# microsoft/DFOL-VQA

Hardware: AMD Instinct MI355X
Metric: questions/sec (GQA programs, N=100 objects) (higher is better)
Workload: dtype f32

## Files before the change

dfol_vqa_amd/csrc/dfol_dense_wide.hip:

```cpp
#include "dfol_common.h"
#include "dfol_split.h"

#include <stdlib.h>

#include <algorithm>
#include <type_traits>

namespace {

constexpr int WD_BM = 128, WD_BK = 32, WD_XD = 3;
constexpr int WD_TILE = 2 * 128 * 4;
constexpr int WD_NMAX = 512;
constexpr size_t WD_LDS = (size_t)6 * WD_TILE * 16 + 2 * WD_NMAX * 4 + 8 * 4096;

template <int ACT, int XV, bool ROWS = false>
__global__ __launch_bounds__(512) __attribute__((amdgpu_waves_per_eu(2, 2))) void wide_h2_kernel(
    const float* __restrict__ X, int64_t ldx, const u32x4* __restrict__ Wp, const float* __restrict__ bias, float* __restrict__ Y, int64_t ldy, int M,
    int N, int K, int ksteps, int nbn, uint32_t* __restrict__ status, const int32_t* __restrict__ src_row) {
    extern __shared__ __attribute__((aligned(16))) u32x4 wd_sm[];
    constexpr int A0 = 0, B0 = 2 * WD_TILE;
    const int tid = threadIdx.x, lane = tid & 63, wave = __builtin_amdgcn_readfirstlane(tid >> 6), kh = lane >> 4, r16 = lane & 15;
    const int wm = wave >> 2, wn = wave & 3;
    const int arow = tid >> 2, aq = tid & 3;
    const int nblocks = (M + WD_BM - 1) / WD_BM, stride = gridDim.x;
    const int first = blockIdx.x;
    if (first >= nblocks) return;
    const int nmine = (nblocks - first + stride - 1) / stride;
    const int T = nmine * ksteps;

    floatx4 acc[4][8];
#pragma unroll
    for (int i = 0; i < 4; ++i)
#pragma unroll
        for (int j = 0; j < 8; ++j) acc[i][j] = floatx4{0.f, 0.f, 0.f, 0.f};

    float4 xa[WD_XD][2];
    int lb = first, lks = 0;
    const int r0 = min(lb * WD_BM + arow, M - 1);
    const float* xrow = X + (int64_t)(ROWS ? src_row[r0] : r0) * ldx + aq * 8;
    auto load_x = [&](auto set_tag) __attribute__((always_inline)) {
        constexpr int S = decltype(set_tag)::value;
        const int k = lks * WD_BK + aq * 8;
        const int c0 = min(k, K - 4) - aq * 8, c1 = min(k + 4, K - 4) - aq * 8;
        auto ld4 = [&](const float* p) __attribute__((always_inline)) {
            if (XV == 4) return *reinterpret_cast<const float4*>(p);
            const float2 lo = *reinterpret_cast<const float2*>(p), hi = *reinterpret_cast<const float2*>(p + 2);
            return make_float4(lo.x, lo.y, hi.x, hi.y);
        };
        xa[S][0] = ld4(xrow + c0);
        xa[S][1] = ld4(xrow + c1);
        if (++lks == ksteps) {
            lks = 0;
            lb += stride;
            const int64_t r = min((int64_t)lb * WD_BM + arow, (int64_t)M - 1);
            xrow = X + (ROWS ? (int64_t)src_row[r] : r) * ldx + aq * 8;
        }
    };
    u32x4 wb[4];
    int wks = 0, wh = 0;
    auto load_w = [&]() __attribute__((always_inline)) {
#pragma unroll
        for (int i = 0; i < 4; ++i) {
            const int idx = i * 512 + tid, nb = 2 * wh + idx / WD_TILE, within = idx % WD_TILE;
            wb[i] = Wp[((int64_t)min(nb, nbn - 1) * ksteps + wks) * WD_TILE + within];
        }
        if (++wh == 2) {
            wh = 0;
            if (++wks == ksteps) wks = 0;
        }
    };
    auto store_b = [&](int buf) __attribute__((always_inline)) {
#pragma unroll
        for (int i = 0; i < 4; ++i) wd_sm[B0 + buf * 2 * WD_TILE + i * 512 + tid] = wb[i];
    };
    float xmax = 0.f;
    int sks = 0;
    auto store_a = [&](auto set_tag, int buf) __attribute__((always_inline)) {
        constexpr int S = decltype(set_tag)::value;
        const int k = sks * WD_BK + aq * 8;
        const int at = A0 + buf * WD_TILE + arow * 4 + (aq ^ dfol_swz(arow));
        const float4 z = make_float4(0.f, 0.f, 0.f, 0.f);
        const float4 v0 = k < K ? xa[S][0] : z, v1 = k + 4 < K ? xa[S][1] : z;
        xmax = fmaxf(fmaxf(xmax, fabsf(v0.x)), fabsf(v0.y));
        xmax = fmaxf(fmaxf(xmax, fabsf(v0.z)), fabsf(v0.w));
        xmax = fmaxf(fmaxf(xmax, fabsf(v1.x)), fabsf(v1.y));
        xmax = fmaxf(fmaxf(xmax, fabsf(v1.z)), fabsf(v1.w));
        u32x4 ph, pl;
        dfol_split2hx8(v0, v1, ph, pl);
        wd_sm[at] = ph;
        wd_sm[at + WD_BM * 4] = pl;
        if (++sks == ksteps) sks = 0;
    };

    const int aoff = (wm * 64 + r16) * 4 + (kh ^ dfol_swz(r16));
    const int boff = (wn >> 1) * WD_TILE + ((wn & 1) * 64 + r16) * 4 + (kh ^ dfol_swz(r16));
    constexpr int PA3[3] = {1, 0, 0}, PB3[3] = {0, 1, 0};
    u32x4 afr[4][2];
    auto load_a = [&](int abuf) __attribute__((always_inline)) {
#pragma unroll
        for (int i = 0; i < 4; ++i)
#pragma unroll
            for (int p = 0; p < 2; ++p) afr[i][p] = wd_sm[A0 + abuf * WD_TILE + aoff + p * WD_BM * 4 + i * 64];
    };
    auto multiply = [&](int bbuf, auto half_tag) __attribute__((always_inline)) {
        constexpr int JB = 4 * decltype(half_tag)::value;
        const int bo = B0 + bbuf * 2 * WD_TILE + boff;
// ... 17 lines not shown
        xs[tid] = tid < nbn * 128 ? tail[tid] : 0.f;
        xs[WD_NMAX + tid] = (bias && tid < N) ? bias[tid] : 0.f;
    }
    float* stage = xs + 2 * WD_NMAX + wave * 1024;
    auto epilogue = [&](int b) __attribute__((always_inline)) {
        const int m0 = b * WD_BM + wm * 64;
#pragma unroll
        for (int h = 0; h < 2; ++h) {
            const int col = h * 256 + wn * 64 + lane;
            const float cs = xs[col], bv = xs[WD_NMAX + col];
            float* yp = Y + col;
#pragma unroll
            for (int i = 0; i < 4; ++i) {
#pragma unroll
                for (int j = 0; j < 4; ++j)
#pragma unroll
                    for (int e = 0; e < 4; ++e) {
                        stage[(4 * kh + e) * 64 + j * 16 + r16] = acc[i][4 * h + j][e];
                        acc[i][4 * h + j][e] = 0.f;
                    }
#pragma unroll 4
                for (int r = 0; r < 16; ++r) {
                    const int row = m0 + i * 16 + r;
                    const float v = dfol_act<ACT>(stage[r * 64 + lane] * cs + bv);
                    if (row < M && col < N) yp[(int64_t)row * ldy] = v;
                }
            }
        }
    };

    const std::integral_constant<int, 0> S0;
    const std::integral_constant<int, 1> S1;
    const std::integral_constant<int, 2> S2;
    load_x(S0);
    load_w();
    load_x(S1);
    load_x(S2);
    store_b(0);
    load_w();
    store_a(S0, 0);
    load_x(S0);
    __syncthreads();
    int g = 0, cks = 0, cb = first;
    auto body = [&](auto next_tag) __attribute__((always_inline)) {
        const int cur = g & 1, nxt = cur ^ 1;
        store_b(1);
        load_w();
        load_a(cur);
        multiply(0, S0);
        __syncthreads();
        store_b(0);
        load_w();
        store_a(next_tag, nxt);
        load_x(next_tag);
        multiply(1, S1);
        __syncthreads();
        ++g;
        if (++cks == ksteps) {
            epilogue(cb);
            cks = 0;
            cb += stride;
        }
    };
    while (g < T) {
        body(S1);
        if (g < T) body(S2);
        if (g < T) body(S0);
    }
    if (status != nullptr && !(xmax <= 65504.0f)) atomicOr(status, (uint32_t)DFOL_RANGE_X_OVERFLOW);
}

int wd_cus() {
    static int cus = 0;
    if (!cus) {
        hipDeviceProp_t prop;
        int dev = 0;
        if (hipGetDevice(&dev) == hipSuccess && hipGetDeviceProperties(&prop, dev) == hipSuccess) cus = prop.multiProcessorCount;
        if (cus <= 0) cus = 256;
    }
    return cus;
}

}

extern "C" int dfol_linear_wide_supported(int64_t M, int32_t N, int32_t K) {
    static const int on = getenv("DFOL_DENSE_WIDE") ? atoi(getenv("DFOL_DENSE_WIDE")) : 1;
    if (!on || N <= 256 || N > WD_NMAX || K < 4 * WD_BK || K % 4 != 0 || M >= (1ll << 31) - 256) return 0;
    if (on != 2 && N <= 384) return 0;
    const int64_t blocks = (M + WD_BM - 1) / WD_BM, rounds = (blocks + wd_cus() - 1) / wd_cus();
    return on == 2 || 4 * blocks >= 3 * rounds * wd_cus();
}

static int wd_launch(const char* name, const float* X, int64_t ldx, const int32_t* src_row, const void* W_split, const float* bias, float* Y, int64_t ldy,
                     int32_t M, int32_t N, int32_t K, int32_t act, void* stream);

extern "C" int dfol_linear_wide_h2_f32(const float* X, int64_t ldx, const void* W_split, const float* bias, float* Y, int64_t ldy, int32_t M, int32_t N,
                                       int32_t K, int32_t act, void* stream) {
    return wd_launch("linear_wide_h2", X, ldx, nullptr, W_split, bias, Y, ldy, M, N, K, act, stream);
}

// ... 42 lines not shown
```

dfol_vqa_amd/_lib.py:

```python

import ctypes
import os
import threading

import torch

_HERE = os.path.dirname(os.path.abspath(__file__))
LIB_PATH = os.environ.get("DFOL_LIB") or os.path.join(_HERE, "libdfolvqa.so")
_lib = None

TILE_SUBJECT_ROWS, TILE_OBJECT_ROWS = 0, 1
WANT_SUBJECT, WANT_OBJECT = 1, 2
RELATE_LONE_FORALL_IDENTITY, RELATE_DIAG_ABSENT = 1, 2
TILE_F32, TILE_BF16 = 0, 1
ACT_NONE, ACT_SIGMOID, ACT_ELU, ACT_LOGSIGMOID = 0, 1, 2, 3
LOGIC_AND, LOGIC_OR, LOGIC_NOT = 0, 1, 2


class DfolError(RuntimeError):
    pass


class LRUCache(object):

# ... 71 lines not shown
    "dfol_segment_or_ref_f32": [_p, _p, _i32, _p, _p],
    "dfol_pair_train_fwd_h2_f32": [_p, _i64, _i32, _p, _i64, _p, _p, _p, _i32, _p, _i64, _p, _p, _p, _i32, _i32, _p, _i32, _p, _p, _i64, _p, _p, _i64, _p],
    "dfol_select_rows_f32": [_p, _p, _p, _i32, _i32, _p, _p],
    "dfol_calib_features_f32": [_p, _i32, _p, _i32, _p, _i32, _p, _p],
    "dfol_attention_modulations_f32": [_p, _p, _p, _i64, _p, _i32, _i32, _i32, _p, _p],
    "dfol_implication_f32": [_p, _p, _p, _p, _i32, _i32, _p, _p],
    "dfol_compare_f32": [_p, _p, _p, _i32, _p, _p],
    "dfol_linear_act_f32": [_p, _i64, _p, _i64, _p, _p, _i64, _i32, _i32, _i32, _i32, _p],
    "dfol_box_positions_f32": [_p, _i64, _i32, _i32, _p, _i64, _i32, _p],
    "dfol_pair_features_f32": [_p, _i64, _i32, _p, _p, _i32, _i32, _p, _i64, _p],
    "dfol_reduce_by_question_f32": [_p, _p, _p, _i32, _i32, _i32, _p, _p],
    "dfol_filter_bwd_f32": [_p, _p, _p, _p, _p, _i32, _p, _i32, _i32, _i32, _p, _p, _p],
    "dfol_relate_bwd_f32": [_p, _p, _p, _p, _p, _p, _p, _p, _i32, _p, _p, _p, _i32, _i32, _i32, _i32, _p, _p, _p, _p],
    "dfol_linear_wgrad_slabs": [_i64, _i32, _i32],
    "dfol_linear_wgrad_f32": [_p, _i64, _p, _i64, _i64, _i32, _i32, _p, _p, _p],
    "dfol_linear_wgrad_workspace": [_i64, _i32, _i32],
    "dfol_linear_wgrad_bias_f32": [_p, _i64, _p, _i64, _i64, _i32, _i32, _p, _p, _p, _p],
    "dfol_attr_ll_bwd_f32": [_p, _p, _i64, _i32, _p, _i64, _p, _p, _p, _p, _i32, _i32, _i32, _p, _p, _i64, _p, _i64, _p, _p],
    "dfol_quantify_bwd_f32": [_p, _p, _p, _p, _p, _i32, _i32, _p, _p],
    "dfol_attr_gather_bwd_f32": [_p, _p, _p, _p, _i32, _i32, _i32, _p, _i64, _p],
    "dfol_rel_gather_bwd_f32": [_p, _p, _p, _p, _p, _i32, _i32, _i32, _i32, _p, _i64, _p],
    "dfol_option_normalize_bwd_f32": [_p, _p, _p, _i32, _p, _p, _i32, _i32, _p, _p],
    "dfol_modulate_f32": [_p, _p, _p, _p, _i32, _i32, _p, _p],
    "dfol_lstm_cell_f32": [_p, _i64, _i32, _p, _i64, _p, _p, _i64, _p, _i64, _p, _p, _i32, _i32, _p, _p, _p],
    "dfol_lstm_cell_tokens_f32": [_p, _i32, _p, _i32, _p, _p, _i64, _p, _p, _i64, _p, _i64, _p, _p, _i32, _i32, _p, _p, _p],
    "dfol_lstm_pointwise_f32": [_p, _p, _p, _i32, _i32, _p, _p, _p],
    "dfol_lstm_cell_train_f32": [_p, _i64, _i32, _p, _i64, _p, _p, _i64, _p, _i64, _p, _p, _i32, _i32, _p, _p, _p, _p],
    "dfol_lstm_cell_bwd_f32": [_p, _p, _p, _p, _p, _i32, _i32, _p, _p, _p],
    "dfol_lstm_cell_supported": [_i32, _i32],
    "dfol_calib_walk_supported": [_i32, _i32],
    "dfol_modulate_bwd_f32": [_p, _p, _p, _p, _p, _i32, _i32, _p, _p, _p],
    "dfol_attr_ll_f32": [_p, _i64, _i32, _p, _i64, _p, _p, _p, _p, _i32, _i32, _f, _p, _p],
    "dfol_attr_head_h2_f32": [_p, _i64, _i32, _p, _p, _i32, _p, _i64, _p, _p, _i32, _i32, _p, _p, _i32, _i32, _f, _p, _p],
    "dfol_pair_ll_f32": [_p, _i64, _i32, _p, _i64, _p, _p, _i64, _i32, _p, _i32, _p, _i64, _p, _p, _p, _i32, _i32, _p, _p, _p, _i32,
                         _i32, _f, _p, _p],
    "dfol_pair_pack_w2_f32": [_p, _i64, _i32, _i32, _p, _p],
    "dfol_pair_ll_packed_f32": [_p, _i64, _i32, _p, _i64, _p, _p, _p, _i32, _p, _i64, _p, _p, _p, _i32, _i32, _p, _p, _p, _i32, _i32, _f,
                                _i32, _p, _p],
    "dfol_pair_hidden1_fwd_f32": [_p, _i64, _p, _i64, _p, _i64, _p, _p, _p, _p, _i32, _i32, _i32, _p, _p, _p],
    "dfol_pair_hidden1_bwd_f32": [_p, _p, _p, _p, _p, _p, _i32, _i32, _i32, _p, _i64, _p, _i64, _p, _p],
    "dfol_pair_hidden1_bwd_recompute_supported": [_i32, _i32],
    "dfol_pair_hidden1_bwd_recompute_f32": [_p, _p, _i64, _p, _i64, _p, _p, _p, _p, _p, _i32, _i32, _i32, _p, _i64, _p, _i64, _p, _p],
    "dfol_pair_logit_fwd_f32": [_p, _i64, _i32, _p, _i64, _p, _p, _i32, _i64, _i64, _p, _p],
    "dfol_pair_logit_bwd_f32": [_p, _p, _i64, _i32, _p, _i64, _p, _i32, _p, _i64, _p, _i64, _p, _p],
    "dfol_pair_logit_bwd_sums_f32": [_p, _p, _i64, _i32, _p, _i64, _p, _i32, _p, _i64, _p, _p, _i64, _p],
    "dfol_linear_tall_supported": [_i64, _i32, _i32],
    "dfol_linear_tall_h2_f32": [_p, _i64, _p, _p, _p, _i64, _i32, _i32, _i32, _p, _p, _i64, _p, _i64, _p],
    "dfol_pair_dz_tall_f32": [_p, _i64, _p, _p, _p, _i64, _p, _p, _p, _i64, _i32, _i32, _i32, _i32, _p, _p],
    "dfol_pair_dz_tall_multi_f32": [_p, _i64, _p, _i64, _i32, _p, _p, _i64, _i32, _p, _p, _p, _i64, _i32, _i32, _i32, _i32, _p, _p],
    "dfol_linear_tall_bf16_bf16": [_p, _i64, _p, _p, _p, _i64, _i32, _i32, _i32, _p, _p, _i64, _p, _i64, _p],
    "dfol_pair_dz_tall_bf16": [_p, _i64, _p, _p, _p, _i64, _p, _p, _i64, _i32, _i32, _i32, _i32, _p],
    "dfol_linear_logit_h2_f32": [_p, _i64, _p, _p, _p, _i64, _i32, _i32, _i32, _p, _p, _i64, _p, _i64, _p],
    "dfol_pair_dz_fused_f32": [_p, _i64, _p, _p, _p, _i64, _p, _p, _p, _i64, _i32, _i32, _i32, _i32, _p],
    "dfol_pair_wgrad_fused_workspace": [_i64, _i32, _i32],
    "dfol_pair_wgrad_fused_sums_workspace": [_i64, _i32, _i32, _i32],
    "dfol_pair_wgrad_fused_sums_f32": [_p, _i64, _p, _p, _p, _i32, _p, _i64, _p, _p, _i64, _i64, _i32, _i32, _p, _p, _p, _i64, _p, _p, _p],
    "dfol_pair_wgrad_fused_sums_bf16": [_p, _i64, _p, _p, _p, _i32, _p, _i64, _p, _i64, _i64, _i32, _i32, _p, _p, _p, _i64, _p, _p, _p],
    "dfol_pair_wgrad_fused_f32": [_p, _i64, _p, _p, _p, _p, _i64, _p, _p, _i64, _i64, _i32, _i32, _p, _p, _p],
    "dfol_pair_wgrad_multi_scale_f32": [_p, _i64, _i32, _p, _p, _i32, _i64, _p, _p],
    "dfol_pair_wgrad_fused_multi_f32": [_p, _i64, _p, _i64, _i32, _p, _p, _p, _i64, _i32, _p, _p, _i64, _i64, _i32, _i32, _p, _p, _p],
    "dfol_linear_pack_w_bf16x3": [_p, _i64, _i32, _i32, _p, _p],
    "dfol_linear_act_split_f32": [_p, _i64, _p, _p, _p, _i64, _i32, _i32, _i32, _i32, _p],
    "dfol_linear_pack_w_bf16": [_p, _i64, _i32, _i32, _p, _p],
    "dfol_linear_act_bf16_f32": [_p, _i64, _p, _p, _p, _i64, _i32, _i32, _i32, _i32, _p],
    "dfol_linear_wgrad_bias_bf16": [_p, _i64, _p, _i64, _i64, _i32, _i32, _p, _p, _p, _p],
    "dfol_linear_wgrad_rows_supported": [_i32, _i32, _i64, _i64],
# ... 1334 lines not shown
```

dfol_vqa_amd/csrc/dfol_pair_h2.hip:

```cpp
#include "dfol_common.h"
#include "dfol_split.h"

#include <stdlib.h>

#include <type_traits>

#ifdef DFOL_PAIR_TRACE
__device__ long long dfol_h2_trace_buf[8 * 8 * 64];
#define TRACE(slot)                                                                                                  \
    do {                                                                                                             \
        if (trace_on && lane == 0) dfol_h2_trace_buf[(trace_blk * 8 + wave) * 64 + (slot)] = clock64();              \
    } while (0)
#else
#define TRACE(slot)
#endif

#ifndef DFOL_H2_PREFETCH
#define DFOL_H2_PREFETCH 1
#endif
#ifndef DFOL_H2_BDEPTH
#define DFOL_H2_BDEPTH 2
#endif
#ifndef DFOL_H1_BDEPTH
#define DFOL_H1_BDEPTH 4
#endif
#ifndef DFOL_H2_DMA_ASM
#define DFOL_H2_DMA_ASM 1
#endif
#ifndef DFOL_H2T_SKIP
#define DFOL_H2T_SKIP 0
#endif
#ifndef DFOL_H2_DMA_LATE
#define DFOL_H2_DMA_LATE 0
#endif


namespace {

constexpr float H2_NL2E = -1.44269504088896340736f;
constexpr int H2_CH = 32;
constexpr int H2_ROWS = 320, H2_TILES = 20;
constexpr int H2_PIECES = 2 * H2_ROWS * 4;
constexpr int H1_PIECES = H2_ROWS * 4;
constexpr float H2_AMAX = 60000.0f;
constexpr float H2_L2E = 1.44269504088896340736f;
constexpr float H2_LN2 = 0.69314718055994530942f;

__device__ __forceinline__ float h2_elu_neg(float zs) {
    const float p = __builtin_amdgcn_fmed3f(__builtin_amdgcn_exp2f(zs), 0.0f, 1.0f);
    return fmaf(p, H2_L2E, -H2_L2E);
}

__host__ __device__ __forceinline__ constexpr int h2_kperm(int kq, int e) { return 16 * (e >> 2) + 4 * kq + (e & 3); }

template <bool HI>
__device__ __forceinline__ float h2_resid(float x, uint32_t hpair) {
    float r;
    if (HI) asm("v_fma_mix_f32 %0, -%1, 1.0, %2 op_sel:[1,0,0] op_sel_hi:[1,0,0]" : "=v"(r) : "v"(hpair), "v"(x));
    else asm("v_fma_mix_f32 %0, -%1, 1.0, %2 op_sel:[0,0,0] op_sel_hi:[1,0,0]" : "=v"(r) : "v"(hpair), "v"(x));
    return r;
}

__global__ void h2_row_scale_kernel(const float* __restrict__ W2, int64_t ld_w2, int HID2, int HID1, float* __restrict__ tail) {
    const int lane = threadIdx.x & 63, r = blockIdx.x * (blockDim.x >> 6) + (threadIdx.x >> 6);
    if (r >= H2_ROWS) return;
    float m = 0.f;
// ... 432 lines not shown
        const float cx = p[0] + p[2] / 2.0f, cy = p[1] + p[3] / 2.0f;
        lox = fminf(lox, cx), hix = fmaxf(hix, cx), loy = fminf(loy, cy), hiy = fmaxf(hiy, cy);
    }
#pragma unroll
    for (int s = 32; s >= 1; s >>= 1) {
        lox = fminf(lox, __shfl_xor(lox, s, 64)), hix = fmaxf(hix, __shfl_xor(hix, s, 64));
        loy = fminf(loy, __shfl_xor(loy, s, 64)), hiy = fmaxf(hiy, __shfl_xor(hiy, s, 64));
    }
    if (lane == 0) box[0][wave] = lox, box[1][wave] = hix, box[2][wave] = loy, box[3][wave] = hiy;
    __syncthreads();
    if (t < HID1) {
#pragma unroll
        for (int w = 0; w < 8; ++w) lox = fminf(lox, box[0][w]), hix = fmaxf(hix, box[1][w]), loy = fminf(loy, box[2][w]), hiy = fmaxf(hiy, box[3][w]);
        const float* pf = reinterpret_cast<const float*>(part);
        float mu = -INFINITY, mv = -INFINITY;
        bool bad = false;
        for (int r = 0; r < R; ++r) {
            const float u = pf[(r * G + t / 4) * 4 + (t & 3)], v = pf[(r * G + (HID1 + t) / 4) * 4 + (t & 3)];
            const float ux = pf[(r * G + t / 4) * 4], vx = pf[(r * G + (HID1 + t) / 4) * 4];
            bad |= (ux != ux) | (vx != vx);
            mu = fmaxf(mu, u), mv = fmaxf(mv, v);
        }
        const float dmax = sqrtf((hix - lox) * (hix - lox) + (hiy - loy) * (hiy - loy));
        const float4 g = *reinterpret_cast<const float4*>(Wg + t * 4);
        const float geo = H2_L2E * (fabsf(g.x) * dmax + fabsf(g.y) * 1.57079632679489661923f + fabsf(g.z) + fabsf(g.w));
        const float bound = mu + mv + geo;
        if (bad || !(bound <= H2_AMAX)) atomicOr(status, (uint32_t)DFOL_RANGE_PAIR_SATURATED);
    }
}


constexpr int AH_WAVES = 4, AH_MT = 2, AH_T = AH_WAVES * 64, AH_SLOTS = AH_WAVES * AH_MT * 16, AH_CAP = 512;

template <int NB16>
__global__ __launch_bounds__(AH_T) void attr_head_h2_kernel(const float* pre1, int64_t ld_pre1, int HID1, const u32x4* __restrict__ W2h,
                                                            const float* __restrict__ b2, int HID2, const float* __restrict__ E, int64_t ld_e,
                                                            const float* __restrict__ be, const int32_t* __restrict__ obj_off, int Q, int O,
                                                            const int32_t* __restrict__ pred_q, const int32_t* __restrict__ pred_col, int P, int NS,
                                                            float dflt, float* __restrict__ ll, uint32_t* __restrict__ status) {
    constexpr int MT = AH_MT, ROWS = NB16 * 16, T = AH_T;
    static_assert(NB16 > 16 && NB16 <= H2_TILES, "geometry");
    __shared__ __attribute__((aligned(16))) u32x4 Bs[2 * H2_PIECES];
    constexpr int STAGE_FLOATS = 8192;
    __shared__ __attribute__((aligned(16))) float stage[STAGE_FLOATS];
    __shared__ int32_t ent[4][AH_CAP];
    __shared__ int ent_n;
    __shared__ int img_cnt[2];
    constexpr int SR = STAGE_FLOATS / ROWS - 2;

    const int tid = threadIdx.x, wave = __builtin_amdgcn_readfirstlane(tid >> 6), lane = tid & 63, kh = lane >> 4, r16 = lane & 15;
    const int nchunk = HID1 / H2_CH;
    const float* cf = reinterpret_cast<const float*>(W2h + (int64_t)nchunk * H2_PIECES);

    auto fill_defaults = [&]() {
        for (int64_t idx = (int64_t)blockIdx.x * T + tid; idx < (int64_t)P * NS; idx += (int64_t)gridDim.x * T) {
            const int p = (int)(idx / NS), o = (int)(idx - (int64_t)p * NS), q = pred_q[p];
            if (pred_col[p] < 0 || o >= obj_off[q + 1] - obj_off[q]) ll[idx] = dflt;
        }
    };
    const int g0 = blockIdx.x * AH_SLOTS;
    if (g0 >= O) {
        fill_defaults();
        return;
    }

    auto dma_chunk = [&](int c, int buf) __attribute__((always_inline)) {
#pragma unroll
        for (int i = 0; i < H2_PIECES / T; ++i)
            __builtin_amdgcn_global_load_lds(W2h + (int64_t)c * H2_PIECES + T * i + tid,
                                             (__attribute__((address_space(3))) void*)&Bs[buf * H2_PIECES + T * i + wave * 64], 16, 0, 0);
    };
    dma_chunk(0, 0);
    const float* row[MT];
#pragma unroll
    for (int m = 0; m < MT; ++m) row[m] = pre1 + (int64_t)min(g0 + wave * (MT * 16) + m * 16 + r16, O - 1) * ld_pre1 + 4 * kh;
    floatx4 ra[MT][2];
    auto load_rows = [&](int c) __attribute__((always_inline)) {
#pragma unroll
        for (int m = 0; m < MT; ++m)
#pragma unroll
            for (int t = 0; t < 2; ++t) ra[m][t] = *reinterpret_cast<const floatx4*>(row[m] + H2_CH * c + 16 * t);
    };
    load_rows(0);
    fill_defaults();
    if (tid < 2) img_cnt[tid] = 0;
    __syncthreads();
    {
        const int g_last = min(g0 + AH_SLOTS, O) - 1;
        int c_lo = 0, c_hi = 0;
        for (int q = 1 + tid; q < Q; q += T) {
            const int f = obj_off[q];
            c_lo += f <= g0, c_hi += f <= g_last;
        }
        if (c_lo) atomicAdd(&img_cnt[0], c_lo);
        if (c_hi) atomicAdd(&img_cnt[1], c_hi);
    }
    for (int i = tid; i < ROWS; i += T) {
        stage[i] = H2_NL2E * (i < HID2 ? b2[i] : -1.0e30f);
        stage[ROWS + i] = i < HID2 ? cf[i] : 0.f;
    }

    floatx4 acc[MT][NB16];
#pragma unroll
    for (int m = 0; m < MT; ++m)
#pragma unroll
        for (int i = 0; i < NB16; ++i) acc[m][i] = floatx4{0.f, 0.f, 0.f, 0.f};
    u32x4 ap[MT][2];
    bool bad = false;
    const int boff = r16 * 4 + (kh ^ dfol_swz(r16));
    constexpr int PA3[3] = {1, 0, 0}, PB3[3] = {0, 1, 0};
    for (int c = 0; c < nchunk; ++c) {
        __builtin_amdgcn_s_waitcnt(0x0F70);
        __syncthreads();
        if (c + 1 < nchunk) dma_chunk(c + 1, (c + 1) & 1);
#pragma unroll
        for (int m = 0; m < MT; ++m)
#pragma unroll
            for (int t = 0; t < 2; ++t)
#pragma unroll
                for (int jp = 0; jp < 2; ++jp) {
                    const float z0 = ra[m][t][2 * jp] * H2_L2E, z1 = ra[m][t][2 * jp + 1] * H2_L2E;
                    bad |= !(z0 <= H2_AMAX) | !(z1 <= H2_AMAX);
                    const float a0 = __builtin_amdgcn_fmed3f(z0, h2_elu_neg(z0), H2_AMAX);
                    const float a1 = __builtin_amdgcn_fmed3f(z1, h2_elu_neg(z1), H2_AMAX);
                    const uint32_t hh = __builtin_bit_cast(uint32_t, __builtin_convertvector((f32x2){a0, a1}, f16x2));
                    const uint32_t lw = __builtin_bit_cast(uint32_t, __builtin_convertvector((f32x2){h2_resid<false>(a0, hh), h2_resid<true>(a1, hh)}, f16x2));
                    ap[m][0][2 * t + jp] = hh;
                    ap[m][1][2 * t + jp] = lw;
                }
        if (c + 1 < nchunk) load_rows(c + 1);
        const int bbase = boff + (c & 1) * H2_PIECES;
        constexpr int D = DFOL_H2_BDEPTH;
        f16x8 bq[D + 1][2];
        auto load_b = [&](int i, f16x8(&b)[2]) __attribute__((always_inline)) {
#pragma unroll
            for (int p = 0; p < 2; ++p) b[p] = __builtin_bit_cast(f16x8, Bs[bbase + i * 64 + p * H2_ROWS * 4]);
        };
#pragma unroll
        for (int d = 0; d < D; ++d) load_b(d, bq[d]);
#pragma unroll
        for (int i = 0; i < NB16; ++i) {
            if (i + D < NB16) load_b(i + D, bq[(i + D) % (D + 1)]);
            __builtin_amdgcn_sched_barrier(0);
#pragma unroll
            for (int m = 0; m < MT; ++m) {
#pragma unroll
                for (int x = 0; x < 3; ++x)
                    acc[m][i] = __builtin_amdgcn_mfma_f32_16x16x32_f16(__builtin_bit_cast(f16x8, ap[m][PA3[x]]), bq[i % (D + 1)][PB3[x]], acc[m][i], 0, 0, 0);
                __builtin_amdgcn_sched_barrier(0);
            }
        }
    }
    if (status && __any(bad) && lane == 0) atomicOr(status, (uint32_t)DFOL_RANGE_X_OVERFLOW);

#pragma unroll
    for (int m = 0; m < MT; ++m)
#pragma unroll
        for (int i = 0; i < NB16; ++i) {
            const float bv = stage[i * 16 + r16], cm = stage[ROWS + i * 16 + r16];
#pragma unroll
            for (int e = 0; e < 4; ++e) acc[m][i][e] = __builtin_amdgcn_rcpf(1.0f + __builtin_amdgcn_exp2f(fmaf(acc[m][i][e], cm, bv)));
        }
    const int q_lo = img_cnt[0], q_hi = img_cnt[1];
    const int w0 = g0 + wave * (MT * 16);
    for (int pw = 0; pw < P; pw += AH_CAP) {
        __syncthreads();
        if (tid == 0) ent_n = 0;
        __syncthreads();
        for (int p = pw + tid; p < min(pw + AH_CAP, P); p += T) {
            const int q = pred_q[p], col = pred_col[p];
            if (col >= 0 && q >= q_lo && q <= q_hi) {
                const int j = atomicAdd(&ent_n, 1);
                ent[0][j] = p, ent[1][j] = col, ent[2][j] = obj_off[q], ent[3][j] = obj_off[q + 1];
            }
        }
        __syncthreads();
        const int n_ent = ent_n;
        if (n_ent == 0) continue;
        const int n_st = n_ent < SR ? n_ent : SR;
        for (int j = 0; j < n_st; ++j) {
            const float* erow = E + (int64_t)ent[1][j] * ld_e;
            for (int i = tid; i < ROWS; i += T) stage[ROWS * (2 + j) + i] = i < HID2 ? erow[i] : 0.f;
        }
        __syncthreads();
        for (int j = 0; j < n_ent; ++j) {
            const int first = __builtin_amdgcn_readfirstlane(ent[2][j]), end = __builtin_amdgcn_readfirstlane(ent[3][j]);
            if (end <= w0 || first >= w0 + MT * 16) continue;
            const int p = __builtin_amdgcn_readfirstlane(ent[0][j]), col = __builtin_amdgcn_readfirstlane(ent[1][j]);
            float vm[MT];
#pragma unroll
            for (int m = 0; m < MT; ++m) {
                float part[4] = {0.f, 0.f, 0.f, 0.f};
                if (j < SR) {
                    const float* erow = stage + ROWS * (2 + j) + r16;
// ... 127 lines not shown
                                          const int32_t* obj_off, const int64_t* pair_off, int32_t Q, int32_t max_n, const int32_t* req_row, int32_t K,
                                          float* Z, float* pre2, int64_t ld_pre2, float* geo, float* x, int64_t ld_x, void* stream) {
    DFOL_REQUIRE(Q >= 0 && K >= 0 && max_n >= 0, "pair_train_fwd_h2: bad sizes Q=%d K=%d max_n=%d", Q, K, max_n);
    DFOL_REQUIRE(HID1 > 0 && HID1 <= 256 && HID1 % H2_CH == 0 && ld_uv % 4 == 0, "pair_train_fwd_h2: HID1=%d must be a multiple of %d, <= 256, UV rows 16-byte aligned", HID1, H2_CH);
    DFOL_REQUIRE(HID2 > 256 && HID2 <= 320 && ld_pre2 >= HID2, "pair_train_fwd_h2: HID2=%d must be in (256, 320], ld_pre2 >= HID2", HID2);
    if (Q == 0 || max_n < 2) return 0;
    DFOL_REQUIRE(UV && pos && Wg && W2_split && b2 && n_obj && obj_off && pair_off && Z && pre2 && geo && (K == 0 || (E && req_row && x)), "pair_train_fwd_h2: null pointer");
    DFOL_REQUIRE(((uintptr_t)UV % 16 == 0) && ((uintptr_t)W2_split % 16 == 0) && ((uintptr_t)Wg % 16 == 0) && ((uintptr_t)Z % 16 == 0) && ((uintptr_t)geo % 16 == 0),
                 "pair_train_fwd_h2: operands must be 16-byte aligned");
    hipStream_t st = (hipStream_t)stream;
    const int tpi = dfol_cdiv((int64_t)max_n * (max_n - 1), 256);
    DFOL_REQUIRE((int64_t)Q * tpi < ((int64_t)1 << 31), "pair_train_fwd_h2: too many tiles");
    DFOL_REQUIRE((int64_t)max_n * ld_uv * 4 < ((int64_t)1 << 31) && (int64_t)max_n * (max_n - 1) * HID1 * 4 < ((int64_t)1 << 32) - 1,
                 "pair_train_fwd_h2: an image's rows must span less than 2 GB (U | V) / 4 GB (Z)");
    if (uint32_t* status = dfol_range_status_ptr())
        hipLaunchKernelGGL(h2_uv_range_kernel, dim3((unsigned)Q), dim3(512), 0, st, UV, ld_uv, HID1, pos, ld_pos, Wg, n_obj, obj_off, status);
    const H2Train tr = {Z, pre2, ld_pre2, geo, x, ld_x, pair_off};
    const int wgt = 1;
    const dim3 grid((unsigned)Q * tpi);
#define DFOL_PAIR32T(NBV)                                                                                                                    \
    hipLaunchKernelGGL((pair_ll32h_kernel<NBV, false, true>), grid, dim3(512), 0, st, UV, ld_uv, HID1, pos, ld_pos, Wg, (const u32x4*)W2_split, b2, HID2, \
                       E, ld_e, (const float*)nullptr, n_obj, obj_off, Q, tpi, wgt, req_row, (const int32_t*)nullptr, (const uint8_t*)nullptr, K, 4, 0.f,      \
                       (void*)nullptr, tr)
    if (HID2 <= 272) DFOL_PAIR32T(17);
    else if (HID2 <= 288) DFOL_PAIR32T(18);
    else if (HID2 <= 304) DFOL_PAIR32T(19);
    else DFOL_PAIR32T(20);
#undef DFOL_PAIR32T
    DFOL_LAUNCH_CHECK("pair_train_fwd_h2");
    return 0;
}


extern "C" int dfol_attr_head_h2_f32(const float* pre1, int64_t ld_pre1, int32_t HID1, const void* W2_split, const float* b2, int32_t HID2,
                                     const float* E, int64_t ld_e, const float* be, const int32_t* obj_off, int32_t Q, int32_t O,
                                     const int32_t* pred_q, const int32_t* pred_col, int32_t P, int32_t NS, float default_ll, float* ll, void* stream) {
    DFOL_REQUIRE(P >= 0 && Q >= 0 && O >= 0 && NS > 0 && NS % 4 == 0, "attr_head_h2: bad sizes P=%d Q=%d O=%d NS=%d", P, Q, O, NS);
    DFOL_REQUIRE(HID1 > 0 && HID1 <= 256 && HID1 % H2_CH == 0 && ld_pre1 % 4 == 0 && ld_pre1 >= HID1,
                 "attr_head_h2: HID1=%d must be a multiple of %d, <= 256, rows 16-byte aligned", HID1, H2_CH);
    DFOL_REQUIRE(HID2 > 256 && HID2 <= 320, "attr_head_h2: HID2=%d must be in (256, 320]", HID2);
    if (P == 0) return 0;
    DFOL_REQUIRE(obj_off && pred_q && pred_col && ll && Q > 0, "attr_head_h2: null pointer (or requests without images)");
    DFOL_REQUIRE(O == 0 || (pre1 && W2_split && b2 && E), "attr_head_h2: null pointer");
    DFOL_REQUIRE(((uintptr_t)pre1 % 16 == 0) && ((uintptr_t)W2_split % 16 == 0), "attr_head_h2: operands must be 16-byte aligned");
    const dim3 grid((unsigned)(O > 0 ? dfol_cdiv(O, AH_SLOTS) : 1));
    uint32_t* status = dfol_range_status_ptr();
#define DFOL_ATTR_HEAD(NBV)                                                                                                                      \
    hipLaunchKernelGGL((attr_head_h2_kernel<NBV>), grid, dim3(AH_T), 0, (hipStream_t)stream, pre1, ld_pre1, HID1, (const u32x4*)W2_split, b2, HID2, E, \
                       ld_e, be, obj_off, Q, O, pred_q, pred_col, P, NS, default_ll, ll, status)
    if (HID2 <= 272) DFOL_ATTR_HEAD(17);
    else if (HID2 <= 288) DFOL_ATTR_HEAD(18);
    else if (HID2 <= 304) DFOL_ATTR_HEAD(19);
    else DFOL_ATTR_HEAD(20);
#undef DFOL_ATTR_HEAD
    DFOL_LAUNCH_CHECK("attr_head_h2");
    return 0;
}
```

include/dfol_vqa.h:

```cpp
#ifndef DFOL_VQA_H
#define DFOL_VQA_H

#include <stdint.h>

#ifdef __cplusplus
extern "C" {
#endif

#define DFOL_ABI_VERSION 3

int dfol_abi_version(void);
const char* dfol_last_error(void);

#define DFOL_TILE_SUBJECT_ROWS 0
#define DFOL_TILE_OBJECT_ROWS 1

#define DFOL_RELATE_LONE_FORALL_IDENTITY 1
#define DFOL_RELATE_DIAG_ABSENT 2
#define DFOL_TILE_F32 0
#define DFOL_TILE_BF16 1
#define DFOL_WANT_SUBJECT 1
#define DFOL_WANT_OBJECT 2

#define DFOL_ACT_NONE 0
// ... 278 lines not shown
int dfol_quantify_bwd_f32(const float* g_lp, const float* att, const float* quant, const int32_t* pred_q, const int32_t* n_obj,
                          int32_t P, int32_t NS, float* g_att, void* stream);

int dfol_attr_gather_bwd_f32(const float* g_ll, const int32_t* obj_off, const int32_t* pred_q, const int32_t* pred_col, int32_t P,
                             int32_t Q, int32_t NS, float* g_table, int64_t ld_table, void* stream);

int dfol_rel_gather_bwd_f32(const float* g_tile, const int64_t* pair_off, const int32_t* n_obj, const int32_t* pred_q,
                            const int32_t* pred_col, int32_t P, int32_t Q, int32_t NS, int32_t orientation, float* g_table,
                            int64_t ld_table, void* stream);

int dfol_attr_ll_bwd_f32(const float* g, const float* hidden, int64_t ld_hidden, int32_t H, const float* E, int64_t ld_e,
                         const float* be, const int32_t* obj_off, const int32_t* pred_q, const int32_t* pred_col, int32_t P,
                         int32_t Q, int32_t NS, float* gx, float* d_hidden, int64_t ld_dh, float* dE, int64_t ld_de, float* db,
                         void* stream);

int dfol_option_normalize_bwd_f32(const float* g_y, const float* y, const int32_t* seg_off, int32_t S, const int32_t* pred_q,
                                  const int32_t* n_obj, int32_t NS, int32_t rank, float* g_x, void* stream);

int32_t dfol_grad_sqnorm_parts(void);
int32_t dfol_clip_adam_chunk(void);
int dfol_grad_sqnorm_f32(const float* g, int64_t n, float* partials, void* stream);
int dfol_clip_adam_f32(float* g, const float* partials, const int64_t* param, const int64_t* exp_avg, const int64_t* exp_avg_sq, const int64_t* goff,
                       const int64_t* numel, int32_t n_tensors, const int32_t* chunk_tensor, const int64_t* chunk_start, int32_t n_chunks,
                       const int64_t* step_ptr, float step_host, float lr, float beta1, float beta2, float eps, float weight_decay, float max_norm,
                       float* norm_out, void* stream);

#define DFOL_RANGE_X_OVERFLOW 1u
#define DFOL_RANGE_PAIR_SATURATED 2u
int dfol_set_range_status(uint32_t* device_word);

int dfol_attr_head_h2_f32(const float* pre1, int64_t ld_pre1, int32_t HID1, const void* W2_split, const float* b2, int32_t HID2, const float* E,
                          int64_t ld_e, const float* be, const int32_t* obj_off, int32_t Q, int32_t O, const int32_t* pred_q,
                          const int32_t* pred_col, int32_t P, int32_t NS, float default_ll, float* ll, void* stream);

#define DFOL_INSTR_WIDTH 16
#define DFOL_DENSE_F32 0
#define DFOL_DENSE_F16X2 1
#define DFOL_DENSE_BF16X3 2
#define DFOL_DENSE_BF16 3
#define DFOL_DENSE_HEAD_F16X2 4
#define DFOL_PAIR_PLAIN 0
#define DFOL_PAIR_PACKED 1
#define DFOL_PAIR_BF16X3 2
#define DFOL_PAIR_F16X2 3
#define DFOL_PAIR_F16 4

typedef struct {
    int32_t kind;
    int32_t act;
    int32_t N, K;
    const float* weight;
    int64_t ldw;
    const void* packed;
    const float* bias;
} DfolDenseLayer;

typedef struct {
    int32_t n_featurizer;
    int32_t n_attribute;
    const DfolDenseLayer* featurizer;
    const DfolDenseLayer* attribute;
    DfolDenseLayer uv;
    int32_t pair_kind;
    int32_t hid1, hid2, w2_rows;
    const float* wg;
    const void* w2;
// ... 71 lines not shown
```

Measured before the change: 193,300.

## Stream weight tiles directly into LDS with global_load_lds and split X loads

Replaces the register-staged weight path (global load into registers, then LDS store) with global_load_lds_dwordx4 DMA straight into the shared B buffers, using manual vmcnt waits. X prefetch loads are split into two halves issued at different pipeline points, with explicit waitcnt handling so the loads overlap the MFMA phases. The goal is to free VGPRs and LDS-store instructions and deepen memory/compute overlap. It relies on hand-tuned vmcnt counts and inline asm ordering, so a miscount could cause hazards.

```diff
diff --git a/dfol_vqa_amd/csrc/dfol_dense_wide.hip b/dfol_vqa_amd/csrc/dfol_dense_wide.hip
--- a/dfol_vqa_amd/csrc/dfol_dense_wide.hip
+++ b/dfol_vqa_amd/csrc/dfol_dense_wide.hip
@@ -38,40 +38,53 @@
     int lb = first, lks = 0;
     const int r0 = min(lb * WD_BM + arow, M - 1);
     const float* xrow = X + (int64_t)(ROWS ? src_row[r0] : r0) * ldx + aq * 8;
-    auto load_x = [&](auto set_tag) __attribute__((always_inline)) {
-        constexpr int S = decltype(set_tag)::value;
-        const int k = lks * WD_BK + aq * 8;
-        const int c0 = min(k, K - 4) - aq * 8, c1 = min(k + 4, K - 4) - aq * 8;
+    int aq8 = aq * 8;
+    auto load_x = [&](auto set_tag, auto part_tag) __attribute__((always_inline)) {
+        constexpr int S = decltype(set_tag)::value, P = decltype(part_tag)::value;
+        const int k = lks * WD_BK + aq8 + 4 * P;
+        const int c = min(k, K - 4) - aq8;
         auto ld4 = [&](const float* p) __attribute__((always_inline)) {
             if (XV == 4) return *reinterpret_cast<const float4*>(p);
             const float2 lo = *reinterpret_cast<const float2*>(p), hi = *reinterpret_cast<const float2*>(p + 2);
             return make_float4(lo.x, lo.y, hi.x, hi.y);
         };
-        xa[S][0] = ld4(xrow + c0);
-        xa[S][1] = ld4(xrow + c1);
-        if (++lks == ksteps) {
+        xa[S][P] = ld4(xrow + c);
+        if (P == 1 && ++lks == ksteps) {
             lks = 0;
             lb += stride;
             const int64_t r = min((int64_t)lb * WD_BM + arow, (int64_t)M - 1);
             xrow = X + (ROWS ? (int64_t)src_row[r] : r) * ldx + aq * 8;
         }
     };
-    u32x4 wb[4];
+    auto wait_x = [&](auto set_tag, auto all_tag) __attribute__((always_inline)) {
+        constexpr int S = decltype(set_tag)::value;
+        floatx4 t0 = {xa[S][0].x, xa[S][0].y, xa[S][0].z, xa[S][0].w}, t1 = {xa[S][1].x, xa[S][1].y, xa[S][1].z, xa[S][1].w};
+        if (decltype(all_tag)::value) asm volatile("s_waitcnt vmcnt(0)" : "+v"(t0), "+v"(t1) : : "memory");
+        else asm volatile("s_waitcnt vmcnt(4)" : "+v"(t0), "+v"(t1));
+        xa[S][0] = make_float4(t0[0], t0[1], t0[2], t0[3]);
+        xa[S][1] = make_float4(t1[0], t1[1], t1[2], t1[3]);
+    };
     int wks = 0, wh = 0;
-    auto load_w = [&]() __attribute__((always_inline)) {
-#pragma unroll
-        for (int i = 0; i < 4; ++i) {
-            const int idx = i * 512 + tid, nb = 2 * wh + idx / WD_TILE, within = idx % WD_TILE;
-            wb[i] = Wp[((int64_t)min(nb, nbn - 1) * ksteps + wks) * WD_TILE + within];
-        }
+    auto dma_b = [&](int buf) __attribute__((always_inline)) {
+        const int nb = min(2 * wh + (wave >> 2), nbn - 1);
+        const u32x4* sp = Wp + ((int64_t)nb * ksteps + wks) * WD_TILE + (wave & 3) * 256 + lane;
+        const uint32_t d = (uint32_t)(uintptr_t)(__attribute__((address_space(3))) void*)(wd_sm + B0 + buf * 2 * WD_TILE + wave * 256);
+        const uint32_t m0v = __builtin_amdgcn_readfirstlane(d);
+#pragma clang diagnostic push
+#pragma clang diagnostic ignored "-Winline-asm"
+        asm volatile("s_mov_b32 m0, %1\n\ts_nop 0\n\tglobal_load_lds_dwordx4 %0, off\n\tglobal_load_lds_dwordx4 %0, off offset:1024\n\t"
+                     "global_load_lds_dwordx4 %0, off offset:2048\n\tglobal_load_lds_dwordx4 %0, off offset:3072" ::"v"(sp), "s"(m0v) : "memory", "m0");
+#pragma clang diagnostic pop
+        asm volatile("" : "+v"(aq8));
         if (++wh == 2) {
             wh = 0;
             if (++wks == ksteps) wks = 0;
         }
     };
-    auto store_b = [&](int buf) __attribute__((always_inline)) {
-#pragma unroll
-        for (int i = 0; i < 4; ++i) wd_sm[B0 + buf * 2 * WD_TILE + i * 512 + tid] = wb[i];
+    auto dma_wait = [&]() __attribute__((always_inline)) {
+        __builtin_amdgcn_sched_barrier(0);
+        asm volatile("s_waitcnt vmcnt(1)" ::: "memory");
+        __builtin_amdgcn_sched_barrier(0);
     };
     float xmax = 0.f;
     int sks = 0;
@@ -155,28 +168,31 @@
     const std::integral_constant<int, 0> S0;
     const std::integral_constant<int, 1> S1;
     const std::integral_constant<int, 2> S2;
-    load_x(S0);
-    load_w();
-    load_x(S1);
-    load_x(S2);
-    store_b(0);
-    load_w();
+    dma_b(0);
+    load_x(S0, S0), load_x(S0, S1);
+    load_x(S1, S0), load_x(S1, S1);
+    load_x(S2, S0), load_x(S2, S1);
+    wait_x(S0, std::true_type());
     store_a(S0, 0);
-    load_x(S0);
+    load_x(S0, S0);
     __syncthreads();
     int g = 0, cks = 0, cb = first;
-    auto body = [&](auto next_tag) __attribute__((always_inline)) {
+    auto body = [&](auto cur_tag, auto next_tag) __attribute__((always_inline)) {
         const int cur = g & 1, nxt = cur ^ 1;
-        store_b(1);
-        load_w();
+        dma_b(1);
+        load_x(cur_tag, S1);
+        __builtin_amdgcn_sched_barrier(0);
         load_a(cur);
         multiply(0, S0);
+        dma_wait();
         __syncthreads();
-        store_b(0);
-        load_w();
+        wait_x(next_tag, std::false_type());
         store_a(next_tag, nxt);
-        load_x(next_tag);
+        dma_b(0);
+        load_x(next_tag, S0);
+        __builtin_amdgcn_sched_barrier(0);
         multiply(1, S1);
+        dma_wait();
         __syncthreads();
         ++g;
         if (++cks == ksteps) {
@@ -186,9 +202,9 @@
         }
     };
     while (g < T) {
-        body(S1);
-        if (g < T) body(S2);
-        if (g < T) body(S0);
+        body(S0, S1);
+        if (g < T) body(S1, S2);
+        if (g < T) body(S2, S0);
     }
     if (status != nullptr && !(xmax <= 65504.0f)) atomicOr(status, (uint32_t)DFOL_RANGE_X_OVERFLOW);
 }
```

New measurement: 193,400, median of 2. About the same (+0.0%).

## Pipeline attr-head H2 kernel with inline-asm LDS DMA and async row loads

Applied to the files above, without the earlier changes.

Adds an ASYNC variant of the attribute-head H2 kernel, on by default. It issues the W2 chunk DMA into LDS through inline-asm global_load_lds_dwordx4 batches using per-wave m0. Row loads are inline-asm global loads waited on explicitly, so the A fragments for the next chunk are built after its MFMAs, overlapping loads with compute instead of a full waitcnt before each barrier. It also adds a 32-bit index path for the default-fill loop and keeps the old kernel as a _ref entry point. The cost is fragile inline assembly with manual waitcnt and m0 handling, plus debug-only lab macros.

```diff
diff --git a/dfol_vqa_amd/_lib.py b/dfol_vqa_amd/_lib.py
--- a/dfol_vqa_amd/_lib.py
+++ b/dfol_vqa_amd/_lib.py
@@ -127,6 +127,7 @@
     "dfol_modulate_bwd_f32": [_p, _p, _p, _p, _p, _i32, _i32, _p, _p, _p],
     "dfol_attr_ll_f32": [_p, _i64, _i32, _p, _i64, _p, _p, _p, _p, _i32, _i32, _f, _p, _p],
     "dfol_attr_head_h2_f32": [_p, _i64, _i32, _p, _p, _i32, _p, _i64, _p, _p, _i32, _i32, _p, _p, _i32, _i32, _f, _p, _p],
+    "dfol_attr_head_h2_ref_f32": [_p, _i64, _i32, _p, _p, _i32, _p, _i64, _p, _p, _i32, _i32, _p, _p, _i32, _i32, _f, _p, _p],
     "dfol_pair_ll_f32": [_p, _i64, _i32, _p, _i64, _p, _p, _i64, _i32, _p, _i32, _p, _i64, _p, _p, _p, _i32, _i32, _p, _p, _p, _i32,
                          _i32, _f, _p, _p],
     "dfol_pair_pack_w2_f32": [_p, _i64, _i32, _i32, _p, _p],
diff --git a/dfol_vqa_amd/csrc/dfol_pair_h2.hip b/dfol_vqa_amd/csrc/dfol_pair_h2.hip
--- a/dfol_vqa_amd/csrc/dfol_pair_h2.hip
+++ b/dfol_vqa_amd/csrc/dfol_pair_h2.hip
@@ -32,6 +32,12 @@
 #endif
 #ifndef DFOL_H2_DMA_LATE
 #define DFOL_H2_DMA_LATE 0
+#endif
+#ifndef DFOL_AH_DMA_ASM
+#define DFOL_AH_DMA_ASM 1
+#endif
+#ifndef DFOL_AH_LAB
+#define DFOL_AH_LAB 0
 #endif
 
 
@@ -530,12 +536,12 @@
 
 constexpr int AH_WAVES = 4, AH_MT = 2, AH_T = AH_WAVES * 64, AH_SLOTS = AH_WAVES * AH_MT * 16, AH_CAP = 512;
 
-template <int NB16>
+template <int NB16, bool ASYNC>
 __global__ __launch_bounds__(AH_T) void attr_head_h2_kernel(const float* pre1, int64_t ld_pre1, int HID1, const u32x4* __restrict__ W2h,
                                                             const float* __restrict__ b2, int HID2, const float* __restrict__ E, int64_t ld_e,
                                                             const float* __restrict__ be, const int32_t* __restrict__ obj_off, int Q, int O,
                                                             const int32_t* __restrict__ pred_q, const int32_t* __restrict__ pred_col, int P, int NS,
-                                                            float dflt, float* __restrict__ ll, uint32_t* __restrict__ status) {
+                                                            float dflt, float* __restrict__ ll, uint32_t* __restrict__ status, int idx32) {
     constexpr int MT = AH_MT, ROWS = NB16 * 16, T = AH_T;
     static_assert(NB16 > 16 && NB16 <= H2_TILES, "geometry");
     __shared__ __attribute__((aligned(16))) u32x4 Bs[2 * H2_PIECES];
@@ -551,6 +557,15 @@
     const float* cf = reinterpret_cast<const float*>(W2h + (int64_t)nchunk * H2_PIECES);
 
     auto fill_defaults = [&]() {
+        if (idx32) {
+            const uint32_t cells = (uint32_t)P * (uint32_t)NS, step = gridDim.x * (uint32_t)T;
+            for (uint32_t idx = blockIdx.x * (uint32_t)T + tid; idx < cells; idx += step) {
+                const uint32_t p = idx / (uint32_t)NS;
+                const int o = (int)(idx - p * (uint32_t)NS), q = pred_q[p];
+                if (pred_col[p] < 0 || o >= obj_off[q + 1] - obj_off[q]) ll[idx] = dflt;
+            }
+            return;
+        }
         for (int64_t idx = (int64_t)blockIdx.x * T + tid; idx < (int64_t)P * NS; idx += (int64_t)gridDim.x * T) {
             const int p = (int)(idx / NS), o = (int)(idx - (int64_t)p * NS), q = pred_q[p];
             if (pred_col[p] < 0 || o >= obj_off[q + 1] - obj_off[q]) ll[idx] = dflt;
@@ -563,10 +578,32 @@
     }
 
     auto dma_chunk = [&](int c, int buf) __attribute__((always_inline)) {
-#pragma unroll
-        for (int i = 0; i < H2_PIECES / T; ++i)
-            __builtin_amdgcn_global_load_lds(W2h + (int64_t)c * H2_PIECES + T * i + tid,
-                                             (__attribute__((address_space(3))) void*)&Bs[buf * H2_PIECES + T * i + wave * 64], 16, 0, 0);
+        if ((DFOL_AH_LAB & 1) && c > 0) return;
+        if constexpr (ASYNC) {
+            constexpr int PER_WAVE = H2_PIECES / AH_WAVES;
+            const u32x4* src = W2h + (int64_t)c * H2_PIECES + wave * PER_WAVE + lane;
+            u32x4* dst = &Bs[buf * H2_PIECES + wave * PER_WAVE];
+#pragma unroll
+            for (int g = 0; g < PER_WAVE / 64; g += 4) {
+                const uint32_t d = (uint32_t)(uintptr_t)(__attribute__((address_space(3))) void*)(dst + 64 * g);
+                const u32x4* sp = src + 64 * g;
+#pragma clang diagnostic push
+#pragma clang diagnostic ignored "-Winline-asm"
+                const uint32_t m0v = __builtin_amdgcn_readfirstlane(d);
+                const int rem = PER_WAVE / 64 - g;
+                if (rem >= 4)
+                    asm volatile("s_mov_b32 m0, %1\n\ts_nop 0\n\tglobal_load_lds_dwordx4 %0, off\n\tglobal_load_lds_dwordx4 %0, off offset:1024\n\t"
+                                 "global_load_lds_dwordx4 %0, off offset:2048\n\tglobal_load_lds_dwordx4 %0, off offset:3072" ::"v"(sp), "s"(m0v) : "memory", "m0");
+                else
+                    asm volatile("s_mov_b32 m0, %1\n\ts_nop 0\n\tglobal_load_lds_dwordx4 %0, off\n\tglobal_load_lds_dwordx4 %0, off offset:1024" ::"v"(sp), "s"(m0v) : "memory", "m0");
+#pragma clang diagnostic pop
+            }
+        } else {
+#pragma unroll
+            for (int i = 0; i < H2_PIECES / T; ++i)
+                __builtin_amdgcn_global_load_lds(W2h + (int64_t)c * H2_PIECES + T * i + tid,
+                                                 (__attribute__((address_space(3))) void*)&Bs[buf * H2_PIECES + T * i + wave * 64], 16, 0, 0);
+        }
     };
     dma_chunk(0, 0);
     const float* row[MT];
@@ -574,10 +611,23 @@
     for (int m = 0; m < MT; ++m) row[m] = pre1 + (int64_t)min(g0 + wave * (MT * 16) + m * 16 + r16, O - 1) * ld_pre1 + 4 * kh;
     floatx4 ra[MT][2];
     auto load_rows = [&](int c) __attribute__((always_inline)) {
-#pragma unroll
-        for (int m = 0; m < MT; ++m)
-#pragma unroll
-            for (int t = 0; t < 2; ++t) ra[m][t] = *reinterpret_cast<const floatx4*>(row[m] + H2_CH * c + 16 * t);
+        if constexpr (ASYNC) {
+            static_assert(MT == 2, "four row registers");
+            const float *p0 = row[0] + H2_CH * c, *p1 = row[1] + H2_CH * c;
+            asm volatile("global_load_dwordx4 %0, %4, off\n\tglobal_load_dwordx4 %1, %4, off offset:64\n\t"
+                         "global_load_dwordx4 %2, %5, off\n\tglobal_load_dwordx4 %3, %5, off offset:64"
+                         : "=&v"(ra[0][0]), "=&v"(ra[0][1]), "=&v"(ra[1][0]), "=&v"(ra[1][1])
+                         : "v"(p0), "v"(p1)
+                         : "memory");
+        } else {
+#pragma unroll
+            for (int m = 0; m < MT; ++m)
+#pragma unroll
+                for (int t = 0; t < 2; ++t) ra[m][t] = *reinterpret_cast<const floatx4*>(row[m] + H2_CH * c + 16 * t);
+        }
+    };
+    auto rows_landed = [&]() __attribute__((always_inline)) {
+        asm volatile("s_waitcnt vmcnt(0)" : "+v"(ra[0][0]), "+v"(ra[0][1]), "+v"(ra[1][0]), "+v"(ra[1][1])::"memory");
     };
     load_rows(0);
     fill_defaults();
@@ -607,10 +657,7 @@
     bool bad = false;
     const int boff = r16 * 4 + (kh ^ dfol_swz(r16));
     constexpr int PA3[3] = {1, 0, 0}, PB3[3] = {0, 1, 0};
-    for (int c = 0; c < nchunk; ++c) {
-        __builtin_amdgcn_s_waitcnt(0x0F70);
-        __syncthreads();
-        if (c + 1 < nchunk) dma_chunk(c + 1, (c + 1) & 1);
+    auto make_a = [&]() __attribute__((always_inline)) {
 #pragma unroll
         for (int m = 0; m < MT; ++m)
 #pragma unroll
@@ -626,7 +673,8 @@
                     ap[m][0][2 * t + jp] = hh;
                     ap[m][1][2 * t + jp] = lw;
                 }
-        if (c + 1 < nchunk) load_rows(c + 1);
+    };
+    auto chunk_mfma = [&](int c) __attribute__((always_inline)) {
         const int bbase = boff + (c & 1) * H2_PIECES;
         constexpr int D = DFOL_H2_BDEPTH;
         f16x8 bq[D + 1][2];
@@ -643,11 +691,41 @@
 #pragma unroll
             for (int m = 0; m < MT; ++m) {
 #pragma unroll
-                for (int x = 0; x < 3; ++x)
+                for (int x = (DFOL_AH_LAB & 2) ? 2 : 0; x < 3; ++x)
                     acc[m][i] = __builtin_amdgcn_mfma_f32_16x16x32_f16(__builtin_bit_cast(f16x8, ap[m][PA3[x]]), bq[i % (D + 1)][PB3[x]], acc[m][i], 0, 0, 0);
                 __builtin_amdgcn_sched_barrier(0);
             }
         }
+    };
+    if constexpr (ASYNC) {
+        rows_landed();
+        make_a();
+        for (int c = 0; c < nchunk; ++c) {
+#pragma unroll
+            for (int m = 0; m < MT; ++m)
+#pragma unroll
+                for (int p = 0; p < 2; ++p) asm volatile("" : "+v"(ap[m][p]));
+            __builtin_amdgcn_sched_barrier(0);
+            __syncthreads();
+            if (c + 1 < nchunk) {
+                dma_chunk(c + 1, (c + 1) & 1);
+                load_rows(c + 1);
+            }
+            chunk_mfma(c);
+            if (c + 1 < nchunk) {
+                rows_landed();
+                make_a();
+            }
+        }
+    } else {
+        for (int c = 0; c < nchunk; ++c) {
+            __builtin_amdgcn_s_waitcnt(0x0F70);
+            __syncthreads();
+            if (c + 1 < nchunk) dma_chunk(c + 1, (c + 1) & 1);
+            make_a();
+            if (c + 1 < nchunk) load_rows(c + 1);
+            chunk_mfma(c);
+        }
     }
     if (status && __any(bad) && lane == 0) atomicOr(status, (uint32_t)DFOL_RANGE_X_OVERFLOW);
 
@@ -657,7 +735,8 @@
         for (int i = 0; i < NB16; ++i) {
             const float bv = stage[i * 16 + r16], cm = stage[ROWS + i * 16 + r16];
 #pragma unroll
-            for (int e = 0; e < 4; ++e) acc[m][i][e] = __builtin_amdgcn_rcpf(1.0f + __builtin_amdgcn_exp2f(fmaf(acc[m][i][e], cm, bv)));
+            for (int e = 0; e < 4; ++e)
+                if (!(DFOL_AH_LAB & 4)) acc[m][i][e] = __builtin_amdgcn_rcpf(1.0f + __builtin_amdgcn_exp2f(fmaf(acc[m][i][e], cm, bv)));
         }
     const int q_lo = img_cnt[0], q_hi = img_cnt[1];
     const int w0 = g0 + wave * (MT * 16);
@@ -851,9 +930,10 @@
 }
 
 
-extern "C" int dfol_attr_head_h2_f32(const float* pre1, int64_t ld_pre1, int32_t HID1, const void* W2_split, const float* b2, int32_t HID2,
-                                     const float* E, int64_t ld_e, const float* be, const int32_t* obj_off, int32_t Q, int32_t O,
-                                     const int32_t* pred_q, const int32_t* pred_col, int32_t P, int32_t NS, float default_ll, float* ll, void* stream) {
+template <bool ASYNC>
+static int attr_head_h2_launch(const float* pre1, int64_t ld_pre1, int32_t HID1, const void* W2_split, const float* b2, int32_t HID2,
+                               const float* E, int64_t ld_e, const float* be, const int32_t* obj_off, int32_t Q, int32_t O,
+                               const int32_t* pred_q, const int32_t* pred_col, int32_t P, int32_t NS, float default_ll, float* ll, void* stream) {
     DFOL_REQUIRE(P >= 0 && Q >= 0 && O >= 0 && NS > 0 && NS % 4 == 0, "attr_head_h2: bad sizes P=%d Q=%d O=%d NS=%d", P, Q, O, NS);
     DFOL_REQUIRE(HID1 > 0 && HID1 <= 256 && HID1 % H2_CH == 0 && ld_pre1 % 4 == 0 && ld_pre1 >= HID1,
                  "attr_head_h2: HID1=%d must be a multiple of %d, <= 256, rows 16-byte aligned", HID1, H2_CH);
@@ -864,9 +944,10 @@
     DFOL_REQUIRE(((uintptr_t)pre1 % 16 == 0) && ((uintptr_t)W2_split % 16 == 0), "attr_head_h2: operands must be 16-byte aligned");
     const dim3 grid((unsigned)(O > 0 ? dfol_cdiv(O, AH_SLOTS) : 1));
     uint32_t* status = dfol_range_status_ptr();
+    const int idx32 = (int64_t)P * NS < (int64_t(1) << 31) && (int64_t)grid.x * AH_T < (int64_t(1) << 31);
 #define DFOL_ATTR_HEAD(NBV)                                                                                                                      \
-    hipLaunchKernelGGL((attr_head_h2_kernel<NBV>), grid, dim3(AH_T), 0, (hipStream_t)stream, pre1, ld_pre1, HID1, (const u32x4*)W2_split, b2, HID2, E, \
-                       ld_e, be, obj_off, Q, O, pred_q, pred_col, P, NS, default_ll, ll, status)
+    hipLaunchKernelGGL((attr_head_h2_kernel<NBV, ASYNC>), grid, dim3(AH_T), 0, (hipStream_t)stream, pre1, ld_pre1, HID1, (const u32x4*)W2_split, b2, \
+                       HID2, E, ld_e, be, obj_off, Q, O, pred_q, pred_col, P, NS, default_ll, ll, status, idx32)
     if (HID2 <= 272) DFOL_ATTR_HEAD(17);
     else if (HID2 <= 288) DFOL_ATTR_HEAD(18);
     else if (HID2 <= 304) DFOL_ATTR_HEAD(19);
@@ -875,3 +956,18 @@
     DFOL_LAUNCH_CHECK("attr_head_h2");
     return 0;
 }
+
+extern "C" int dfol_attr_head_h2_f32(const float* pre1, int64_t ld_pre1, int32_t HID1, const void* W2_split, const float* b2, int32_t HID2,
+                                     const float* E, int64_t ld_e, const float* be, const int32_t* obj_off, int32_t Q, int32_t O,
+                                     const int32_t* pred_q, const int32_t* pred_col, int32_t P, int32_t NS, float default_ll, float* ll, void* stream) {
+    return attr_head_h2_launch<DFOL_AH_DMA_ASM != 0>(pre1, ld_pre1, HID1, W2_split, b2, HID2, E, ld_e, be, obj_off, Q, O, pred_q, pred_col, P, NS,
+                                                     default_ll, ll, stream);
+}
+
+extern "C" int dfol_attr_head_h2_ref_f32(const float* pre1, int64_t ld_pre1, int32_t HID1, const void* W2_split, const float* b2, int32_t HID2,
+                                         const float* E, int64_t ld_e, const float* be, const int32_t* obj_off, int32_t Q, int32_t O,
+                                         const int32_t* pred_q, const int32_t* pred_col, int32_t P, int32_t NS, float default_ll, float* ll,
+                                         void* stream) {
+    return attr_head_h2_launch<false>(pre1, ld_pre1, HID1, W2_split, b2, HID2, E, ld_e, be, obj_off, Q, O, pred_q, pred_col, P, NS, default_ll, ll,
+                                      stream);
+}
diff --git a/include/dfol_vqa.h b/include/dfol_vqa.h
--- a/include/dfol_vqa.h
+++ b/include/dfol_vqa.h
@@ -334,6 +334,9 @@
 int dfol_attr_head_h2_f32(const float* pre1, int64_t ld_pre1, int32_t HID1, const void* W2_split, const float* b2, int32_t HID2, const float* E,
                           int64_t ld_e, const float* be, const int32_t* obj_off, int32_t Q, int32_t O, const int32_t* pred_q,
                           const int32_t* pred_col, int32_t P, int32_t NS, float default_ll, float* ll, void* stream);
+int dfol_attr_head_h2_ref_f32(const float* pre1, int64_t ld_pre1, int32_t HID1, const void* W2_split, const float* b2, int32_t HID2, const float* E,
+                              int64_t ld_e, const float* be, const int32_t* obj_off, int32_t Q, int32_t O, const int32_t* pred_q,
+                              const int32_t* pred_col, int32_t P, int32_t NS, float default_ll, float* ll, void* stream);
 
 #define DFOL_INSTR_WIDTH 16
 #define DFOL_DENSE_F32 0
```

New measurement: 195,300 before, 194,500 after. About the same (-0.4%).
